# teamtomo/torch-motion-correction

Hardware: NVIDIA B200
Metric: movies_per_second_estimate_plus_correct (higher is better)
Workload: dtype f32

## Files before the change

torch_motion_correction_b200/csrc/fourier.cu:

```cuda
#include "common.cuh"
#include <stdlib.h>
#include "fft_core.cuh"
#include "fft_core2.cuh"

namespace {

using tmcfft::pad_idx;
using tmcfft::padded_len;

constexpr int kThreads = 256;

__host__ __device__ constexpr int batch_for(int n) { return n >= 4096 ? 1 : (4096 / n > 16 ? 16 : 4096 / n); }

template <int N>
constexpr size_t fft_smem_bytes() {
  return 2ull * batch_for(N) * padded_len(N) * sizeof(float2);
}


inline bool pow2_n(int n) { return n >= 16 && n <= 8192 && (n & (n - 1)) == 0; }
inline int fft_size_for(int n) {
  if (pow2_n(n)) return n;
  if (n < 2) return 0;
  int m = 16;
// ... 716 lines not shown
                        rows_per_cta));
        } else {
          if (int e = enable_smem(poly::rows_forward_poly<2>, poly::smem_bytes)) return e;
          TMC_TIMED("rows_forward_poly<2>", stream,
                    poly::rows_forward_poly<2><<<grid, poly::kThreads, poly::smem_bytes, stream>>>(
                        image, h, w, mean_std, mask, jobs, frame_shifts, x_margin, ylo, yhi, ny, kx_count, px.tw, (float2*)tmp,
                        rows_per_cta));
        }
        return TMC_OK;
      }
    }
    if constexpr ((MM == 8192 || MM == 4096) && !BB) {
      if (yhi > ylo && job_mode == 2 && px.R == 1 && kx_count <= MM / 2 && use_real2n(MM)) {
        constexpr int NH = MM / 2;
        constexpr int B = fft2::Cfg<NH>::B;
        int rows_per_cta = B * 4;
        while (rows_per_cta > B && (long)tmc_div_up(yhi - ylo, rows_per_cta) * njobs < 148 * 8) rows_per_cta -= B;
        dim3 grid(tmc_div_up(yhi - ylo, rows_per_cta), njobs);
        constexpr size_t smem = rows_forward_real2n_smem_bytes<NH>();
        if (int e = enable_smem(rows_forward_real2n<NH>, smem)) return e;
        TMC_TIMED(MM == 8192 ? "rows_forward_real2n<4096>" : "rows_forward_real2n<2048>", stream,
                  rows_forward_real2n<NH><<<grid, fft2::kThreads, smem, stream>>>(image, h, w, mean_std, mask, jobs, frame_shifts, x_margin,
                                                                                   ylo, yhi, ny, kx_count, px.tw, (float2*)tmp,
                                                                                   rows_per_cta));
        return TMC_OK;
      }
    }
    if constexpr (use_fast_path<MM, BB>()) if (px.R == 1) {
      if (yhi > ylo) {
        constexpr int B = fft2::Cfg<MM>::B;
        int rows_per_cta = B * 4;
        while (rows_per_cta > B && (long)tmc_div_up(yhi - ylo, rows_per_cta) * njobs < 148 * 8) rows_per_cta -= B;
        dim3 grid(tmc_div_up(yhi - ylo, rows_per_cta), njobs);
        constexpr size_t smem = rows_forward_smem_bytes<MM>();
#define TMC_ROWS_FWD(MODE)                                                                                      \
  {                                                                                                             \
    if (int e = enable_smem(rows_forward_p2<MM, MODE>, smem)) return e;                                         \
    tmc_timing_begin(stream);                                                                                   \
    rows_forward_p2<MM, MODE><<<grid, fft2::kThreads, smem, stream>>>(image, h, w, mean_std, mask, jobs, frame_shifts, \
                                                                     x_margin, ylo, yhi, ny, kx_count, px.tw,          \
                                                                     (float2*)tmp, rows_per_cta);                      \
    tmc_timing_end(MM == 4096 ? "rows_forward_p2<4096>" : "rows_forward_p2", stream);                            \
  }
        if (job_mode == 1) TMC_ROWS_FWD(1) else if (job_mode == 2) TMC_ROWS_FWD(2) else TMC_ROWS_FWD(0)
#undef TMC_ROWS_FWD
        tmc_count_launch();
      }
      return TMC_OK;
    }
    const size_t smem = fft_smem_bytes<MM>() + (px.R > 1 ? 2ull * batch_for(MM) * kx_count * sizeof(float2) : 0);
    if (smem > kMaxSmem) {
      tmc_set_error("rfft2_band: band of %d bins too wide for the decimated row transform of length %d", kx_count, nx);
      return TMC_ERR_UNSUPPORTED;
    }
    if (int e = enable_smem(rows_forward_kernel<MM, BB>, smem)) return e;
    dim3 grid(tmc_div_up(yhi - ylo, batch_for(MM)), njobs);
    if (yhi > ylo) {
      TMC_TIMED("rows_forward_kernel", stream, rows_forward_kernel<MM, BB><<<grid, kThreads, smem, stream>>>(
          image, h, w, mean_std, mask, jobs, frame_shifts, x_margin, ylo, yhi, ny, kx_count, px, (float2*)tmp));
    }
    return TMC_OK;
  });
}

}


TMC_API int tmc_fft_supported_length(int n) {
  if (fft_size_for(n) > 0) return 1;
  const int R = decimation_for(n);
  if (R == 0) return 0;
  return decimated_full_fits(n) ? 1 : 2;
}

TMC_API long tmc_fft_plan_elems(int n_total) {
  const int R = decimation_for(n_total);
  if (R == 0) return 0;
  const int n = n_total / R;
  const int m = fft_size_for(n);
  return m == n ? (long)m : 2l * m + n;
}

TMC_API int tmc_fft_plan_init(int n_total, void* plan, cudaStream_t stream) {
  TMC_CHECK_ARG(plan, "fft_plan_init: null pointer");
  const int R = decimation_for(n_total);
  if (R == 0) {
    tmc_set_error("fft_plan_init: transform length %d is not supported", n_total);
    return TMC_ERR_UNSUPPORTED;
  }
  const int n = n_total / R;
  const int m = fft_size_for(n);
  float2* tw = (float2*)plan;
  TMC_TIMED("twiddle_kernel", stream, twiddle_kernel<<<tmc_div_up(m, 128), 128, 0, stream>>>(m, tw));
  if (m != n) {
    float2* chirp = tw + m;
    float2* bhat = chirp + n;
    TMC_TIMED("chirp_kernel", stream, chirp_kernel<<<tmc_div_up(m, 128), 128, 0, stream>>>(n, m, chirp, bhat));
    AxisPlan p;
    p.tw = tw;
    p.chirp = nullptr;
    p.bhat = nullptr;
    p.n = m;
    p.R = 1;
    p.n_total = m;
    int rc = dispatch_fft(m, "fft_plan_init", [&](auto M, auto) {
      constexpr int MM = decltype(M)::value;
      if (int e = enable_smem(c2c_rows_kernel<MM, false>, fft_smem_bytes<MM>())) return e;
      TMC_TIMED("c2c_rows_kernel", stream, c2c_rows_kernel<MM, false><<<1, kThreads, fft_smem_bytes<MM>(), stream>>>(bhat, 1, p, bhat));
      return TMC_OK;
    });
    if (rc) return rc;
  }
  TMC_CHECK_LAUNCH("tmc_fft_plan_init");
  return TMC_OK;
}

TMC_API int tmc_fft_c2c_rows(const void* in, int rows, int n, const void* plan, void* out, cudaStream_t stream) {
  TMC_CHECK_ARG(in && out && plan && rows >= 1, "fft_c2c_rows: bad arguments");
  TMC_CHECK_ARG(fft_size_for(n) > 0, "fft_c2c_rows: full transforms need lengths up to 4096 or powers of two up to 8192, got %d", n);
  AxisPlan p = make_axis_plan(plan, n);
  int rc = dispatch_fft(n, "fft_c2c_rows", [&](auto M, auto BLU) {
    constexpr int MM = decltype(M)::value;
    constexpr bool BB = decltype(BLU)::value;
    if (int e = enable_smem(c2c_rows_kernel<MM, BB>, fft_smem_bytes<MM>())) return e;
    TMC_TIMED("c2c_rows_kernel", stream, c2c_rows_kernel<MM, BB><<<tmc_div_up(rows, batch_for(MM)), kThreads, fft_smem_bytes<MM>(), stream>>>(
        (const float2*)in, rows, p, (float2*)out));
    return TMC_OK;
  });
  if (rc) return rc;
  TMC_CHECK_LAUNCH("tmc_fft_c2c_rows");
  return TMC_OK;
}

TMC_API int tmc_rfft2_band(const float* image, int t, int h, int w, const float* mean_std, const float* mask, int ny, int nx,
                           const int* jobs, int njobs, int job_mode, const int* frame_shifts, int x_margin, int ylo, int yhi,
                           int kx_count, int ky_count, int ky_start, const float* weight, const void* plan_x,
                           const void* plan_y, void* tmp, void* out, cudaStream_t stream) {
  TMC_CHECK_ARG(image && jobs && plan_x && plan_y && tmp && out, "rfft2_band: null pointer");
  TMC_CHECK_ARG(job_mode >= 0 && job_mode <= 2, "rfft2_band: job_mode must be 0 (generic), 1 (mask powers 1,2 of one frame) or 2 (two frames)");
  TMC_CHECK_ARG(njobs >= 0 && t >= 1 && h >= ny && w >= nx, "rfft2_band: window (%d,%d) larger than image (%d,%d)", ny, nx, h, w);
  TMC_CHECK_ARG(0 <= ylo && ylo <= yhi && yhi <= ny, "rfft2_band: bad row support [%d,%d)", ylo, yhi);
  TMC_CHECK_ARG(x_margin >= 0 && 2 * x_margin <= nx, "rfft2_band: bad x_margin %d", x_margin);
  TMC_CHECK_ARG(kx_count >= 1 && kx_count <= nx / 2 + 1 && ky_count >= 1 && ky_count <= ny, "rfft2_band: bad band box");
  if (njobs == 0) return TMC_OK;
  const AxisPlan px = make_axis_plan(plan_x, nx), py = make_axis_plan(plan_y, ny);
  int rc = rfft2_rows(image, h, w, mean_std, mask, ny, nx, jobs, njobs, job_mode, frame_shifts, x_margin, ylo, yhi, kx_count,
                      px, tmp, stream);
  if (rc) return rc;
  TMC_CHECK_LAUNCH("tmc_rfft2_band(rows)");
  rc = dispatch_fft(ny, "rfft2_band", [&](auto M, auto BLU) {
    constexpr int MM = decltype(M)::value;
    constexpr bool BB = decltype(BLU)::value;
    if constexpr (use_fast_path<MM, BB>()) if (py.R == 1) {
      if (int e = enable_smem(cols_forward_p2<MM>, fft2::Cfg<MM>::smem_bytes)) return e;
      dim3 grid(tmc_div_up(kx_count, fft2::Cfg<MM>::B), 2 * njobs);
      TMC_TIMED(sized_label<MM>("cols_forward_p2<4096>", "cols_forward_p2<1024>", "cols_forward_p2"), stream, cols_forward_p2<MM><<<grid, fft2::kThreads, fft2::Cfg<MM>::smem_bytes, stream>>>(
          (const float2*)tmp, ylo, yhi, kx_count, ky_count, ky_start, weight, py.tw, (float2*)out));
      return TMC_OK;
    }
    const size_t smem = fft_smem_bytes<MM>() + (py.R > 1 ? 1ull * batch_for(MM) * ky_count * sizeof(float2) : 0);
    if (smem > kMaxSmem) {
      tmc_set_error("rfft2_band: band of %d bins too wide for the decimated column transform of length %d", ky_count, ny);
      return TMC_ERR_UNSUPPORTED;
    }
    if (int e = enable_smem(cols_forward_kernel<MM, BB>, smem)) return e;
    dim3 grid(tmc_div_up(kx_count, batch_for(MM)), 2 * njobs);
    TMC_TIMED("cols_forward_kernel", stream, cols_forward_kernel<MM, BB><<<grid, kThreads, smem, stream>>>(
                  (const float2*)tmp, ylo, yhi, kx_count, ky_count, ky_start, weight, py, (float2*)out));
    return TMC_OK;
  });
  if (rc) return rc;
  TMC_CHECK_LAUNCH("tmc_rfft2_band(cols)");
  return TMC_OK;
}

__global__ void integer_shifts_kernel(const float* __restrict__ field, int t, float scale, int* __restrict__ shifts,
                                      int* __restrict__ not_integer) {
  const int f = blockIdx.x * blockDim.x + threadIdx.x;
  if (f >= t) return;
  const float sy = scale * field[f], sx = scale * field[t + f];
  const float ry = rintf(sy), rx = rintf(sx);
  shifts[2 * f] = (int)ry;
  shifts[2 * f + 1] = (int)rx;
  if (!(fabsf(sy - ry) <= 1e-4f && fabsf(sx - rx) <= 1e-4f && fabsf(ry) < 1e6f && fabsf(rx) < 1e6f)) *not_integer = 1;
}

TMC_API int tmc_integer_shifts(const float* field, int t, float scale, int* shifts, int* not_integer, cudaStream_t stream) {
  TMC_CHECK_ARG(field && shifts && not_integer && t >= 1, "integer_shifts: bad arguments");
  TMC_CUDA(cudaMemsetAsync(not_integer, 0, sizeof(int), stream));
  TMC_TIMED("integer_shifts_kernel", stream, integer_shifts_kernel<<<tmc_div_up(t, 128), 128, 0, stream>>>(field, t, scale, shifts, not_integer));
  TMC_CHECK_LAUNCH("tmc_integer_shifts");
  return TMC_OK;
}

TMC_API int tmc_xc_pair_products(const void* spec, const int* ref_plane, const int* cur_plane, int nitems, long plane_elems,
                                 void* out, cudaStream_t stream) {
  TMC_CHECK_ARG(spec && ref_plane && cur_plane && out && nitems >= 0 && plane_elems >= 1, "xc_pair_products: bad arguments");
  if (nitems == 0) return TMC_OK;
  dim3 grid((unsigned)(tmc_div_up(plane_elems, 256) < 64 ? tmc_div_up(plane_elems, 256) : 64), nitems);
  TMC_TIMED("xc_pair_product_kernel", stream, xc_pair_product_kernel<<<grid, 256, 0, stream>>>((const float2*)spec, ref_plane, cur_plane, plane_elems, (float2*)out));
  TMC_CHECK_LAUNCH("tmc_xc_pair_products");
  return TMC_OK;
}

TMC_API int tmc_xc_leave_one_out_products(const void* spec, int t, int g, long plane_elems, const int* delta_offsets,
                                          const int* deltas, int k_begin, int k_count, void* out, cudaStream_t stream) {
  TMC_CHECK_ARG(spec && delta_offsets && deltas && out && t >= 2 && g >= 1 && plane_elems >= 1,
                "xc_leave_one_out_products: bad arguments (need t >= 2)");
  TMC_CHECK_ARG(k_begin >= 0 && k_count >= 0 && k_begin + k_count <= t, "xc_leave_one_out_products: bad frame range");
  if (k_count == 0) return TMC_OK;
  dim3 grid(tmc_div_up(plane_elems, 128), g);
  TMC_TIMED("xc_leave_one_out_kernel", stream, xc_leave_one_out_kernel<<<grid, 128, 0, stream>>>((const float2*)spec, t, g, plane_elems, delta_offsets, deltas,
                                                    k_begin, k_count, (float2*)out));
  TMC_CHECK_LAUNCH("tmc_xc_leave_one_out_products");
  return TMC_OK;
}

TMC_API int tmc_xc_peak_partials(int ny, int nx) {
  const int R = decimation_for(nx);
  if (R == 0) return -1;
  const int m = fft_size_for(nx / R);
  if (R == 1 && m == nx && m >= 256) {
    const int b = 256 / (m / 16) > 0 ? 256 / (m / 16) : 1;
    if (m == 8192 || m == 4096) {
      const int bh = 256 / (m / 32) > 0 ? 256 / (m / 32) : 1;
      return tmc_div_up(ny, bh * kRowIters);
    }
    return tmc_div_up(ny, 2 * b * kRowIters);
  }
  return tmc_div_up(ny, 2 * batch_for(m));
}

TMC_API int tmc_xc_peaks(const void* prod, int nitems, int ny, int nx, int kx_count, int ky_count, int ky_start,
                         int sub_pixel, const void* plan_x, const void* plan_y, void* tmp, void* partial, float* shifts,
                         cudaStream_t stream) {
  TMC_CHECK_ARG(prod && plan_x && plan_y && tmp && partial && shifts, "xc_peaks: null pointer");
  TMC_CHECK_ARG(kx_count >= 1 && kx_count <= nx / 2 + 1 && ky_count >= 1 && ky_count <= ny, "xc_peaks: bad band box");
  if (nitems == 0) return TMC_OK;
  const AxisPlan px = make_axis_plan(plan_x, nx), py = make_axis_plan(plan_y, ny);
  int rc = dispatch_fft(ny, "xc_peaks", [&](auto M, auto BLU) {
    constexpr int MM = decltype(M)::value;
    constexpr bool BB = decltype(BLU)::value;
    if constexpr (use_fast_path<MM, BB>()) if (py.R == 1) {
      if (int e = enable_smem(cols_inverse_p2<MM>, fft2::Cfg<MM>::smem_bytes)) return e;
      dim3 grid(tmc_div_up(kx_count, fft2::Cfg<MM>::B), nitems);
      TMC_TIMED(sized_label<MM>("cols_inverse_p2<4096>", "cols_inverse_p2<1024>", "cols_inverse_p2"), stream, cols_inverse_p2<MM><<<grid, fft2::kThreads, fft2::Cfg<MM>::smem_bytes, stream>>>(
          (const float2*)prod, kx_count, ky_count, ky_start, py.tw, (float2*)tmp));
      return TMC_OK;
    }
    if (int e = enable_smem(cols_inverse_kernel<MM, BB>, fft_smem_bytes<MM>())) return e;
    dim3 grid(tmc_div_up(kx_count, batch_for(MM)), nitems);
    TMC_TIMED("cols_inverse_kernel", stream, cols_inverse_kernel<MM, BB><<<grid, kThreads, fft_smem_bytes<MM>(), stream>>>((const float2*)prod, kx_count, ky_count, ky_start,
                                                                                 py, (float2*)tmp));
    return TMC_OK;
  });
  if (rc) return rc;
  TMC_CHECK_LAUNCH("tmc_xc_peaks(cols)");
  int nparts = tmc_xc_peak_partials(ny, nx);
  rc = dispatch_fft(nx, "xc_peaks", [&](auto M, auto BLU) {
    constexpr int MM = decltype(M)::value;
    constexpr bool BB = decltype(BLU)::value;
    if constexpr ((MM == 8192 || MM == 4096) && !BB) {
      if (px.R == 1 && kx_count <= MM / 4 && use_real2n(MM)) {
        constexpr int NH = MM / 2;
        if (int e = enable_smem(rows_inverse_argmax_real2n<NH>, rows_inverse_real2n_smem_bytes<NH>())) return e;
        nparts = tmc_div_up(ny, rows_per_cta_inverse_real2n<NH>());
        dim3 grid(nparts, nitems);
        TMC_TIMED(MM == 8192 ? "rows_inverse_argmax_real2n<4096>" : "rows_inverse_argmax_real2n<2048>", stream,
                  rows_inverse_argmax_real2n<NH><<<grid, fft2::kThreads, rows_inverse_real2n_smem_bytes<NH>(), stream>>>(
                      (const float2*)tmp, ny, kx_count, px.tw, (PeakCandidate*)partial));
        return TMC_OK;
      }
      nparts = tmc_div_up(ny, rows_per_cta_inverse<MM>());
    }
    if constexpr (MM == 1024 && !BB) {
      if (kx_count <= 128 && use_poly() && px.R == 1) {
        if (int e = enable_smem(poly::rows_inverse_argmax_poly, poly::smem_bytes)) return e;
        dim3 grid(nparts, nitems);
        TMC_TIMED("rows_inverse_argmax_poly", stream, poly::rows_inverse_argmax_poly<<<grid, poly::kThreads, poly::smem_bytes, stream>>>((const float2*)tmp, ny, kx_count, px.tw,
                                                                                         (PeakCandidate*)partial));
        return TMC_OK;
      }
    }
    if constexpr (use_fast_path<MM, BB>()) if (px.R == 1) {
      if (int e = enable_smem(rows_inverse_argmax_p2<MM>, rows_inverse_smem_bytes<MM>())) return e;
      dim3 grid(nparts, nitems);
      TMC_TIMED(sized_label<MM>("rows_inverse_argmax_p2<4096>", "rows_inverse_argmax_p2<1024>", "rows_inverse_argmax_p2"), stream, rows_inverse_argmax_p2<MM><<<grid, fft2::kThreads, rows_inverse_smem_bytes<MM>(), stream>>>(
          (const float2*)tmp, ny, kx_count, px.tw, (PeakCandidate*)partial));
      return TMC_OK;
    }
    if (int e = enable_smem(rows_inverse_argmax_kernel<MM, BB>, fft_smem_bytes<MM>())) return e;
    dim3 grid(nparts, nitems);
    TMC_TIMED("rows_inverse_argmax_kernel", stream, rows_inverse_argmax_kernel<MM, BB><<<grid, kThreads, fft_smem_bytes<MM>(), stream>>>((const float2*)tmp, ny, kx_count, px,
                                                                                        (PeakCandidate*)partial));
    return TMC_OK;
  });
  if (rc) return rc;
  TMC_CHECK_LAUNCH("tmc_xc_peaks(rows)");
  TMC_TIMED("peak_finalize_kernel", stream, peak_finalize_kernel<<<nitems, 128, 0, stream>>>((const float2*)tmp, (const PeakCandidate*)partial, nparts, ny, nx,
                                                   kx_count, sub_pixel, shifts));
  TMC_CHECK_LAUNCH("tmc_xc_peaks(finalize)");
  return TMC_OK;
}

namespace {

int irfft2_cols(const void* spec, int nitems, int ny, int KX, int KY, int ky_start, const AxisPlan& py, void* tmp,
                cudaStream_t stream, const char* who) {
  return dispatch_fft(ny, who, [&](auto M, auto BLU) {
    constexpr int MM = decltype(M)::value;
// ... 202 lines not shown
```

torch_motion_correction_b200/csrc/fourier_p2.cuh:

```cuda
#pragma once


__device__ __forceinline__ void cp_async_f32(float* smem_dst, const float* gmem_src) {
  const unsigned dst = (unsigned)__cvta_generic_to_shared(smem_dst);
  asm volatile("cp.async.ca.shared.global [%0], [%1], 4;\n" ::"r"(dst), "l"(gmem_src));
}
__device__ __forceinline__ void cp_async_commit_and_wait() {
  asm volatile("cp.async.commit_group;\n" ::);
  asm volatile("cp.async.wait_group 0;\n" ::: "memory");
}

template <int N>
constexpr size_t rows_forward_smem_bytes() {
  return fft2::Cfg<N>::smem_bytes + 3ull * fft2::Cfg<N>::B * N * sizeof(float);
}

template <int N, int MODE>
__global__ void __launch_bounds__(fft2::kThreads, N == 4096 ? 2 : 1)
rows_forward_p2(const float* __restrict__ image, int H, int W, const float* __restrict__ mean_std,
                const float* __restrict__ mask, const int* __restrict__ jobs, const int* __restrict__ frame_shifts,
                int x_margin, int ylo, int yhi, int NY, int KX, const float2* __restrict__ tw, float2* __restrict__ tmp,
                int rows_per_cta) {
  using C = fft2::Cfg<N>;
  using P = fft2::Plan<N>;
  extern __shared__ float2 smem[];
  const fft2::Smem<N> sm(smem);
  fft2::load_twiddles<N>(sm, tw);
  const int seq = threadIdx.x / C::TPS, j = threadIdx.x % C::TPS;
  float2* myseq = sm.data + seq * C::STRIDE;
  float* stage_a = reinterpret_cast<float*>(smem + C::B * C::STRIDE + 64 + C::TW_HI);
  float* stage_b = stage_a + C::B * N;
  float* stage_m = stage_b + C::B * N;
  const int job = blockIdx.y;
  const int fa = jobs[job * 6 + 0], ea = jobs[job * 6 + 1], fb = jobs[job * 6 + 2], eb = jobs[job * 6 + 3];
  const int y0 = jobs[job * 6 + 4], x0 = jobs[job * 6 + 5];
  float mean = 0.f, inv_std = 1.f;
  if (mean_std != nullptr) {
    mean = __ldg(mean_std);
    inv_std = 1.0f / __ldg(mean_std + 1);
  }
  const Window wa = make_window(image, fa, y0, x0, frame_shifts, H, W, ylo, yhi, N, x_margin);
  const Window wb = make_window(image, fb >= 0 ? fb : fa, y0, x0, frame_shifts, H, W, ylo, yhi, N, x_margin);
  const float* img_a = wa.fast_base(W);
  const bool has_b = fb >= 0;
  const bool separate_b = has_b && (MODE == 2 || (MODE == 0 && fb != fa));
  const float* img_b = wb.fast_base(W);
  const int row_begin = ylo + blockIdx.x * rows_per_cta;
  const int row_end = min(yhi, row_begin + rows_per_cta);
  float2* plane_a = tmp + (long)(2 * job) * NY * KX;
  float2* plane_b = plane_a + (long)NY * KX;

  auto prefetch = [&](int row0) {
    const int y = row0 + seq;
    if (y < row_end) {
#pragma unroll
      for (int e = 0; e < C::VPT; ++e) {
        const int x = P::First::in_index(j, e / P::First::R, e % P::First::R);
        const int slot = e * fft2::kThreads + threadIdx.x;
        cp_async_f32(stage_a + slot, wa.wrap ? wa.wrapped(y, x, H, W) : img_a + (long)y * W + x);
        if (separate_b) cp_async_f32(stage_b + slot, wb.wrap ? wb.wrapped(y, x, H, W) : img_b + (long)y * W + x);
        if (mask) cp_async_f32(stage_m + slot, mask + (long)y * N + x);
      }
    }
  };
  prefetch(row_begin);
  __syncthreads();
  for (int row0 = row_begin; row0 < row_end; row0 += C::B) {
    const int y = row0 + seq;
    const bool active = y < row_end;
    cp_async_commit_and_wait();
    float2 v[C::VPT];
#pragma unroll
    for (int e = 0; e < C::VPT; ++e) {
      float2 z = make_float2(0.f, 0.f);
      if (active) {
        const int slot = e * fft2::kThreads + threadIdx.x;
        const float m = mask ? stage_m[slot] : 1.0f;
        const float pa = (stage_a[slot] - mean) * inv_std;
        if (MODE == 1) {
          z.x = pa * m;
          z.y = z.x * m;
        } else if (MODE == 2) {
          z.x = pa * m;
          if (has_b) z.y = (stage_b[slot] - mean) * inv_std * m;
        } else {
          float va = pa;
          for (int k = 0; k < ea; ++k) va *= m;
          z.x = va;
          if (has_b) {
            float vb = separate_b ? (stage_b[slot] - mean) * inv_std : pa;
            for (int k = 0; k < eb; ++k) vb *= m;
            z.y = vb;
          }
        }
      }
      v[e] = z;
    }
    if (row0 + C::B < row_end) prefetch(row0 + C::B);
    fft2::fft_regs_to_regs<N>(sm, myseq, j, v);
    __syncthreads();
    P::Last::store(myseq, j, v);
    __syncthreads();
    if (active) {
      for (int k = j; k < KX; k += C::TPS) {
        const float2 zk = myseq[fft2::pad_idx(k)];
        const float2 zn = myseq[fft2::pad_idx(k == 0 ? 0 : N - k)];
        plane_a[(long)y * KX + k] = make_float2(0.5f * (zk.x + zn.x), 0.5f * (zk.y - zn.y));
        if (has_b) plane_b[(long)y * KX + k] = make_float2(0.5f * (zk.y + zn.y), -0.5f * (zk.x - zn.x));
      }
    }
    __syncthreads();
  }
}

__device__ __forceinline__ void cp_async_f32x2_any(float2* smem_dst, const float2* gmem_src) {
  const unsigned dst = (unsigned)__cvta_generic_to_shared(smem_dst);
  asm volatile("cp.async.ca.shared.global [%0], [%1], 8;\n" ::"r"(dst), "l"(gmem_src));
}

template <int N>
constexpr size_t rows_forward_real2n_smem_bytes() {
  return fft2::Cfg<N>::smem_bytes + 2ull * fft2::Cfg<N>::B * N * sizeof(float2);
}

template <int N>
__global__ void __launch_bounds__(fft2::kThreads, N >= 2048 ? 2 : 1)
rows_forward_real2n(const float* __restrict__ image, int H, int W, const float* __restrict__ mean_std,
                    const float* __restrict__ mask, const int* __restrict__ jobs, const int* __restrict__ frame_shifts,
                    int x_margin, int ylo, int yhi, int NY, int KX, const float2* __restrict__ tw2n,
                    float2* __restrict__ tmp, int rows_per_cta) {
  using C = fft2::Cfg<N>;
  using P = fft2::Plan<N>;
  extern __shared__ float2 smem[];
  const fft2::Smem<N> sm(smem);
  for (int i = threadIdx.x; i < 64 + C::TW_HI; i += fft2::kThreads)
    sm.tw_lo[i] = i < 64 ? __ldg(tw2n + 2 * i) : __ldg(tw2n + 2 * (i - 64) * 64);
  const int seq = threadIdx.x / C::TPS, j = threadIdx.x % C::TPS;
  float2* myseq = sm.data + seq * C::STRIDE;
  float2* stage_p = smem + C::B * C::STRIDE + 64 + C::TW_HI;
  float2* stage_m = stage_p + C::B * N;
  const int job = blockIdx.y;
  const int fa = jobs[job * 6 + 0], fb = jobs[job * 6 + 2];
  const int y0 = jobs[job * 6 + 4], x0 = jobs[job * 6 + 5];
  float mean = 0.f, inv_std = 1.f;
  if (mean_std != nullptr) {
    mean = __ldg(mean_std);
    inv_std = 1.0f / __ldg(mean_std + 1);
  }
  const Window wa = make_window(image, fa, y0, x0, frame_shifts, H, W, ylo, yhi, 2 * N, x_margin);
  const Window wb = make_window(image, fb >= 0 ? fb : fa, y0, x0, frame_shifts, H, W, ylo, yhi, 2 * N, x_margin);
  const int halves = fb >= 0 ? 2 : 1;
  const int row_begin = ylo + blockIdx.x * rows_per_cta;
  const int row_end = min(yhi, row_begin + rows_per_cta);
  const int nunits = row_end > row_begin ? ((row_end - row_begin + C::B - 1) / C::B) * halves : 0;
  float2* plane_a = tmp + (long)(2 * job) * NY * KX;

  auto prefetch = [&](int u) {
    const int y = row_begin + (u / halves) * C::B + seq;
    if (y >= row_end) return;
    const bool second = (u % halves) == 1;
    const Window& wd = second ? wb : wa;
    const float* row = wd.fast_base(W) + (long)y * W;
    const bool pair_ok = !wd.wrap && (reinterpret_cast<uintptr_t>(row) & 7) == 0;
#pragma unroll
    for (int e = 0; e < C::VPT; ++e) {
      const int x = 2 * P::First::in_index(j, e / P::First::R, e % P::First::R);
      const int slot = e * fft2::kThreads + threadIdx.x;
      if (pair_ok) {
        cp_async_f32x2_any(stage_p + slot, reinterpret_cast<const float2*>(row + x));
      } else {
        float* dst = reinterpret_cast<float*>(stage_p + slot);
        cp_async_f32(dst, wd.wrap ? wd.wrapped(y, x, H, W) : row + x);
        cp_async_f32(dst + 1, wd.wrap ? wd.wrapped(y, x + 1, H, W) : row + x + 1);
      }
      if (mask && !second) cp_async_f32x2_any(stage_m + slot, reinterpret_cast<const float2*>(mask + (long)y * (2 * N) + x));
    }
  };
  if (nunits > 0) prefetch(0);
  __syncthreads();
  for (int u = 0; u < nunits; ++u) {
    const int y = row_begin + (u / halves) * C::B + seq;
    const bool active = y < row_end;
    const bool second = (u % halves) == 1;
    cp_async_commit_and_wait();
    float2 v[C::VPT];
#pragma unroll
    for (int e = 0; e < C::VPT; ++e) {
      float2 z = make_float2(0.f, 0.f);
      if (active) {
        const int slot = e * fft2::kThreads + threadIdx.x;
        const float2 px = stage_p[slot];
        const float2 m = mask ? stage_m[slot] : make_float2(1.f, 1.f);
        z.x = (px.x - mean) * inv_std * m.x;
        z.y = (px.y - mean) * inv_std * m.y;
      }
      v[e] = z;
    }
    if (u + 1 < nunits) prefetch(u + 1);
    fft2::fft_regs_to_regs<N>(sm, myseq, j, v);
    __syncthreads();
    P::Last::store(myseq, j, v);
    __syncthreads();
    if (active) {
      float2* plane = plane_a + (second ? (long)NY * KX : 0l);
      for (int k = j; k < KX; k += C::TPS) {
        const float2 zk = myseq[fft2::pad_idx(k)];
        const float2 zn = myseq[fft2::pad_idx(k == 0 ? 0 : N - k)];
        const float2 ev = make_float2(0.5f * (zk.x + zn.x), 0.5f * (zk.y - zn.y));
        const float2 od = make_float2(0.5f * (zk.y + zn.y), -0.5f * (zk.x - zn.x));
        plane[(long)y * KX + k] = cadd(ev, cmul(__ldg(tw2n + k), od));
      }
    }
    __syncthreads();
  }
}

template <int N>
__global__ void __launch_bounds__(fft2::kThreads)
cols_forward_p2(const float2* __restrict__ tmp, int ylo, int yhi, int KX, int KY, int ky_start,
                const float* __restrict__ weight, const float2* __restrict__ tw, float2* __restrict__ out) {
  using C = fft2::Cfg<N>;
  using P = fft2::Plan<N>;
  extern __shared__ float2 smem[];
  const fft2::Smem<N> sm(smem);
  fft2::load_twiddles<N>(sm, tw);
  const int seq = threadIdx.x % C::B, j = threadIdx.x / C::B;
  float2* myseq = sm.data + seq * C::STRIDE;
  const long plane = blockIdx.y;
  const int kx = blockIdx.x * C::B + seq;
  const bool active = kx < KX;
  const float2* src = tmp + plane * N * KX + kx;
  float2 v[C::VPT];
#pragma unroll
  for (int g = 0; g < P::First::G; ++g)
#pragma unroll
    for (int r = 0; r < P::First::R; ++r) {
      const int y = P::First::in_index(j, g, r);
      v[g * P::First::R + r] = (active && y >= ylo && y < yhi) ? src[(long)y * KX] : make_float2(0.f, 0.f);
    }
  __syncthreads();
  fft2::fft_regs_to_regs<N>(sm, myseq, j, v);
  if (!active) return;
  float2* dst = out + plane * KY * KX + kx;
#pragma unroll
  for (int g = 0; g < P::Last::G; ++g)
#pragma unroll
    for (int r = 0; r < P::Last::R; ++r) {
      const int ky = P::Last::out_index(j, g, r);
      const int kyb = (ky - ky_start) & (N - 1);
      if (kyb < KY) {
        float2 val = P::Last::result(v, g, r);
        if (weight) {
          const float wgt = __ldg(weight + (long)kyb * KX + kx);
          val.x *= wgt;
          val.y *= wgt;
        }
        dst[(long)kyb * KX] = val;
      }
    }
}

template <int N>
__global__ void __launch_bounds__(fft2::kThreads)
cols_inverse_p2(const float2* __restrict__ in, int KX, int KY, int ky_start, const float2* __restrict__ tw,
                float2* __restrict__ tmp) {
  using C = fft2::Cfg<N>;
  using P = fft2::Plan<N>;
  extern __shared__ float2 smem[];
  const fft2::Smem<N> sm(smem);
  fft2::load_twiddles<N>(sm, tw);
  const int seq = threadIdx.x % C::B, j = threadIdx.x / C::B;
  float2* myseq = sm.data + seq * C::STRIDE;
  const long item = blockIdx.y;
  const int kx = blockIdx.x * C::B + seq;
  const bool active = kx < KX;
  const float2* src = in + item * KY * KX + kx;
  float2 v[C::VPT];
#pragma unroll
  for (int g = 0; g < P::First::G; ++g)
#pragma unroll
    for (int r = 0; r < P::First::R; ++r) {
      const int y = P::First::in_index(j, g, r);
      const int kyb = (y - ky_start) & (N - 1);
      float2 z = make_float2(0.f, 0.f);
      if (active && kyb < KY) {
        const float2 c = src[(long)kyb * KX];
        z = make_float2(c.y, c.x);
      }
      v[g * P::First::R + r] = z;
    }
  __syncthreads();
  fft2::fft_regs_to_regs<N>(sm, myseq, j, v);
  if (!active) return;
  float2* dst = tmp + item * N * KX + kx;
#pragma unroll
  for (int g = 0; g < P::Last::G; ++g)
#pragma unroll
    for (int r = 0; r < P::Last::R; ++r) {
      const float2 val = P::Last::result(v, g, r);
      dst[(long)P::Last::out_index(j, g, r) * KX] = make_float2(val.y, val.x);
    }
}


__device__ __forceinline__ void cp_async_f32x2(float2* smem_dst, const float2* gmem_src) {
  const unsigned dst = (unsigned)__cvta_generic_to_shared(smem_dst);
  asm volatile("cp.async.ca.shared.global [%0], [%1], 8;\n" ::"r"(dst), "l"(gmem_src));
}

constexpr int kRowIters = 4;

template <int N>
__host__ __device__ constexpr int rows_per_cta_inverse() {
  return 2 * fft2::Cfg<N>::B * kRowIters;
}

template <int N>
constexpr size_t rows_inverse_smem_bytes() {
  return fft2::Cfg<N>::smem_bytes + 2ull * fft2::Cfg<N>::B * N * sizeof(float2);
}

template <int N>
__device__ __forceinline__ int c2r_source_index(int i, int KX) {
  if (i < KX) return i;
  const int k = N - i;
  return (k < KX && 2 * k != N) ? k : -1;
}

template <int N>
__device__ __forceinline__ float2 c2r_pack(float2 ca, float2 cb, int i, int KX) {
  if (i < KX) {
    if (i == 0 || 2 * i == N) return make_float2(cb.x, ca.x);
    return make_float2(ca.y + cb.x, ca.x - cb.y);
  }
  return make_float2(cb.x - ca.y, ca.x + cb.y);
}

template <int N, typename Consume>
__device__ __forceinline__ void rows_inverse_driver(const float2* __restrict__ src, int NY, int KX,
                                                    const float2* __restrict__ tw, float2* smem, Consume&& consume) {
  using C = fft2::Cfg<N>;
  using P = fft2::Plan<N>;
  const fft2::Smem<N> sm(smem);
  fft2::load_twiddles<N>(sm, tw);
  const int seq = threadIdx.x / C::TPS, j = threadIdx.x % C::TPS;
  float2* myseq = sm.data + seq * C::STRIDE;
  float2* stage_a = smem + C::B * C::STRIDE + 64 + C::TW_HI;
  float2* stage_b = stage_a + C::B * N;
  auto row_of = [&](int it) { return (int)blockIdx.x * rows_per_cta_inverse<N>() + (it * C::B + seq) * 2; };
  auto prefetch = [&](int it) {
    const int ya = row_of(it);
    if (ya >= NY) return;
    const float2* rowa = src + (long)ya * KX;
    const bool has_b = ya + 1 < NY;
#pragma unroll
    for (int e = 0; e < C::VPT; ++e) {
      constexpr int R = P::First::R;
      const int lo = (e / R) * C::TPS + (e % R) * P::First::NBR;
      if (lo >= KX && lo + C::TPS <= N - KX + 1) continue;
      const int k = c2r_source_index<N>(P::First::in_index(j, e / R, e % R), KX);
      if (k >= 0) {
        const int slot = e * fft2::kThreads + threadIdx.x;
        cp_async_f32x2(stage_a + slot, rowa + k);
        if (has_b) cp_async_f32x2(stage_b + slot, rowa + KX + k);
      }
    }
  };
  prefetch(0);
  __syncthreads();
  for (int it = 0; it < kRowIters; ++it) {
    const int ya = row_of(it);
    const bool active = ya < NY;
    const bool has_b = ya + 1 < NY;
    cp_async_commit_and_wait();
    float2 v[C::VPT];
#pragma unroll
    for (int e = 0; e < C::VPT; ++e) {
      constexpr int R = P::First::R;
      float2 z = make_float2(0.f, 0.f);
      const int lo = (e / R) * C::TPS + (e % R) * P::First::NBR;
      if (active && !(lo >= KX && lo + C::TPS <= N - KX + 1)) {
        const int i = P::First::in_index(j, e / R, e % R);
        if (c2r_source_index<N>(i, KX) >= 0) {
          const int slot = e * fft2::kThreads + threadIdx.x;
          z = c2r_pack<N>(stage_a[slot], has_b ? stage_b[slot] : make_float2(0.f, 0.f), i, KX);
        }
      }
      v[e] = z;
    }
    if (it + 1 < kRowIters) prefetch(it + 1);
    fft2::fft_regs_to_regs<N>(sm, myseq, j, v);
    if (active) consume(ya, has_b, j, v);
    __syncthreads();
  }
}

template <int N>
__global__ void __launch_bounds__(fft2::kThreads, N == 4096 ? 3 : 1)
rows_inverse_argmax_p2(const float2* __restrict__ tmp, int NY, int KX, const float2* __restrict__ tw,
                       PeakCandidate* __restrict__ partial) {
  using P = fft2::Plan<N>;
  extern __shared__ float2 smem[];
  const long item = blockIdx.y;
  float best = -INFINITY;
  int best_idx = 0x7fffffff;
  rows_inverse_driver<N>(tmp + item * NY * KX, NY, KX, tw, smem, [&](int ya, bool has_b, int j, const float2* v) {
#pragma unroll
    for (int r = 0; r < P::Last::R; ++r)
#pragma unroll
      for (int g = 0; g < P::Last::G; ++g) {
        const float val = P::Last::result(v, g, r).y;
        if (val > best) {
          best = val;
          best_idx = ya * N + P::Last::out_index(j, g, r);
        }
      }
    if (has_b) {
#pragma unroll
      for (int r = 0; r < P::Last::R; ++r)
#pragma unroll
        for (int g = 0; g < P::Last::G; ++g) {
          const float val = P::Last::result(v, g, r).x;
          if (val > best) {
            best = val;
            best_idx = (ya + 1) * N + P::Last::out_index(j, g, r);
          }
        }
    }
  });
#pragma unroll
  for (int o = 16; o > 0; o >>= 1) {
    const float ov = __shfl_xor_sync(0xffffffffu, best, o);
    const int oi = __shfl_xor_sync(0xffffffffu, best_idx, o);
    if (better(ov, oi, best, best_idx)) {
      best = ov;
      best_idx = oi;
    }
  }
  __shared__ float sval[fft2::kThreads / 32];
  __shared__ int sidx[fft2::kThreads / 32];
  if ((threadIdx.x & 31) == 0) {
    sval[threadIdx.x >> 5] = best;
    sidx[threadIdx.x >> 5] = best_idx;
  }
  __syncthreads();
  if (threadIdx.x == 0) {
    for (int i = 1; i < fft2::kThreads / 32; ++i)
      if (better(sval[i], sidx[i], best, best_idx)) {
        best = sval[i];
        best_idx = sidx[i];
      }
    PeakCandidate c;
    c.val = best;
    c.idx = best_idx;
    partial[item * gridDim.x + blockIdx.x] = c;
  }
}

template <int N>
__host__ __device__ constexpr int rows_per_cta_inverse_real2n() {
  return fft2::Cfg<N>::B * kRowIters;
// ... 351 lines not shown
```

Baseline: 51.65.

## Make forward column FFT persistent over groups with cp.async prefetch staging

The forward column FFT kernel now handles several column groups per CTA, up to four when N<=4096. While it transforms the current group, it prefetches the next group's column data into a shared-memory staging buffer with cp.async. The goal is to hide global-load latency behind FFT compute and to reuse the twiddle load across groups. In exchange it uses more shared memory, raises the minimum blocks per SM in launch bounds, and launches fewer CTAs, which could reduce parallelism on small problems.

```diff
diff --git a/torch_motion_correction_b200/csrc/fourier.cu b/torch_motion_correction_b200/csrc/fourier.cu
--- a/torch_motion_correction_b200/csrc/fourier.cu
+++ b/torch_motion_correction_b200/csrc/fourier.cu
@@ -892,10 +892,11 @@
     constexpr int MM = decltype(M)::value;
     constexpr bool BB = decltype(BLU)::value;
     if constexpr (use_fast_path<MM, BB>()) if (py.R == 1) {
-      if (int e = enable_smem(cols_forward_p2<MM>, fft2::Cfg<MM>::smem_bytes)) return e;
-      dim3 grid(tmc_div_up(kx_count, fft2::Cfg<MM>::B), 2 * njobs);
-      TMC_TIMED(sized_label<MM>("cols_forward_p2<4096>", "cols_forward_p2<1024>", "cols_forward_p2"), stream, cols_forward_p2<MM><<<grid, fft2::kThreads, fft2::Cfg<MM>::smem_bytes, stream>>>(
-          (const float2*)tmp, ylo, yhi, kx_count, ky_count, ky_start, weight, py.tw, (float2*)out));
+      constexpr size_t smem = cols_forward_smem_bytes<MM>();
+      if (int e = enable_smem(cols_forward_p2<MM>, smem)) return e;
+      const long ngroups = (long)tmc_div_up(kx_count, fft2::Cfg<MM>::B) * 2 * njobs;
+      TMC_TIMED(sized_label<MM>("cols_forward_p2<4096>", "cols_forward_p2<1024>", "cols_forward_p2"), stream, cols_forward_p2<MM><<<tmc_div_up(ngroups, cols_forward_groups<MM>()), fft2::kThreads, smem, stream>>>(
+          (const float2*)tmp, ylo, yhi, kx_count, ky_count, ky_start, ngroups, weight, py.tw, (float2*)out));
       return TMC_OK;
     }
     const size_t smem = fft_smem_bytes<MM>() + (py.R > 1 ? 1ull * batch_for(MM) * ky_count * sizeof(float2) : 0);
diff --git a/torch_motion_correction_b200/csrc/fourier_p2.cuh b/torch_motion_correction_b200/csrc/fourier_p2.cuh
--- a/torch_motion_correction_b200/csrc/fourier_p2.cuh
+++ b/torch_motion_correction_b200/csrc/fourier_p2.cuh
@@ -8,6 +8,11 @@
 __device__ __forceinline__ void cp_async_commit_and_wait() {
   asm volatile("cp.async.commit_group;\n" ::);
   asm volatile("cp.async.wait_group 0;\n" ::: "memory");
+}
+
+__device__ __forceinline__ void cp_async_f32x2(float2* smem_dst, const float2* gmem_src) {
+  const unsigned dst = (unsigned)__cvta_generic_to_shared(smem_dst);
+  asm volatile("cp.async.ca.shared.global [%0], [%1], 8;\n" ::"r"(dst), "l"(gmem_src));
 }
 
 template <int N>
@@ -216,48 +221,90 @@
 }
 
 template <int N>
-__global__ void __launch_bounds__(fft2::kThreads)
-cols_forward_p2(const float2* __restrict__ tmp, int ylo, int yhi, int KX, int KY, int ky_start,
+__host__ __device__ constexpr bool cols_forward_staged() {
+  return N <= 4096;
+}
+
+template <int N>
+__host__ __device__ constexpr int cols_forward_groups() {
+  return cols_forward_staged<N>() ? 4 : 1;
+}
+
+template <int N>
+constexpr size_t cols_forward_smem_bytes() {
+  return fft2::Cfg<N>::smem_bytes + (cols_forward_staged<N>() ? (size_t)fft2::Cfg<N>::VPT * fft2::kThreads * sizeof(float2) : 0);
+}
+
+template <int N>
+__global__ void __launch_bounds__(fft2::kThreads, cols_forward_staged<N>() ? 3 : 2)
+cols_forward_p2(const float2* __restrict__ tmp, int ylo, int yhi, int KX, int KY, int ky_start, long ngroups,
                 const float* __restrict__ weight, const float2* __restrict__ tw, float2* __restrict__ out) {
+  constexpr bool STAGED = cols_forward_staged<N>();
   using C = fft2::Cfg<N>;
   using P = fft2::Plan<N>;
   extern __shared__ float2 smem[];
   const fft2::Smem<N> sm(smem);
   fft2::load_twiddles<N>(sm, tw);
+  float2* stage = smem + C::B * C::STRIDE + 64 + C::TW_HI;
   const int seq = threadIdx.x % C::B, j = threadIdx.x / C::B;
   float2* myseq = sm.data + seq * C::STRIDE;
-  const long plane = blockIdx.y;
-  const int kx = blockIdx.x * C::B + seq;
-  const bool active = kx < KX;
-  const float2* src = tmp + plane * N * KX + kx;
-  float2 v[C::VPT];
-#pragma unroll
-  for (int g = 0; g < P::First::G; ++g)
-#pragma unroll
-    for (int r = 0; r < P::First::R; ++r) {
-      const int y = P::First::in_index(j, g, r);
-      v[g * P::First::R + r] = (active && y >= ylo && y < yhi) ? src[(long)y * KX] : make_float2(0.f, 0.f);
-    }
-  __syncthreads();
-  fft2::fft_regs_to_regs<N>(sm, myseq, j, v);
-  if (!active) return;
-  float2* dst = out + plane * KY * KX + kx;
-#pragma unroll
-  for (int g = 0; g < P::Last::G; ++g)
-#pragma unroll
-    for (int r = 0; r < P::Last::R; ++r) {
-      const int ky = P::Last::out_index(j, g, r);
-      const int kyb = (ky - ky_start) & (N - 1);
-      if (kyb < KY) {
-        float2 val = P::Last::result(v, g, r);
-        if (weight) {
-          const float wgt = __ldg(weight + (long)kyb * KX + kx);
-          val.x *= wgt;
-          val.y *= wgt;
+  const int gx = (KX + C::B - 1) / C::B;
+  const long u0 = (long)blockIdx.x * cols_forward_groups<N>();
+  const int nu = (int)min((long)cols_forward_groups<N>(), ngroups - u0);
+  auto prefetch = [&](long u) {
+    if constexpr (!STAGED) return;
+    const long plane = u / gx;
+    const int kx = (int)(u - plane * gx) * C::B + seq;
+    if (kx >= KX) return;
+    const float2* src = tmp + plane * N * KX + kx;
+#pragma unroll
+    for (int g = 0; g < P::First::G; ++g)
+#pragma unroll
+      for (int r = 0; r < P::First::R; ++r) {
+        const int y = P::First::in_index(j, g, r);
+        if (y >= ylo && y < yhi) cp_async_f32x2(stage + (g * P::First::R + r) * fft2::kThreads + threadIdx.x, src + (long)y * KX);
+      }
+  };
+  prefetch(u0);
+  for (int i = 0; i < nu; ++i) {
+    const long u = u0 + i;
+    const long plane = u / gx;
+    const int kx = (int)(u - plane * gx) * C::B + seq;
+    const bool active = kx < KX;
+    if (STAGED) cp_async_commit_and_wait();
+    const float2* src = tmp + plane * N * KX + kx;
+    float2 v[C::VPT];
+#pragma unroll
+    for (int g = 0; g < P::First::G; ++g)
+#pragma unroll
+      for (int r = 0; r < P::First::R; ++r) {
+        const int y = P::First::in_index(j, g, r);
+        v[g * P::First::R + r] = !(active && y >= ylo && y < yhi) ? make_float2(0.f, 0.f)
+                                 : STAGED ? stage[(g * P::First::R + r) * fft2::kThreads + threadIdx.x]
+                                          : src[(long)y * KX];
+      }
+    if (i + 1 < nu) prefetch(u + 1);
+    __syncthreads();
+    fft2::fft_regs_to_regs<N>(sm, myseq, j, v);
+    if (!active) continue;
+    float2* dst = out + plane * KY * KX + kx;
+#pragma unroll
+    for (int g = 0; g < P::Last::G; ++g)
+#pragma unroll
+      for (int r = 0; r < P::Last::R; ++r) {
+        const int ky = P::Last::out_index(j, g, r);
+        const int kyb = (ky - ky_start) & (N - 1);
+        if (kyb < KY) {
+          float2 val = P::Last::result(v, g, r);
+          if (weight) {
+            const float wgt = __ldg(weight + (long)kyb * KX + kx);
+            val.x *= wgt;
+            val.y *= wgt;
+          }
+          dst[(long)kyb * KX] = val;
         }
-        dst[(long)kyb * KX] = val;
-      }
-    }
+      }
+  }
 }
 
 template <int N>
@@ -302,11 +349,6 @@
     }
 }
 
-
-__device__ __forceinline__ void cp_async_f32x2(float2* smem_dst, const float2* gmem_src) {
-  const unsigned dst = (unsigned)__cvta_generic_to_shared(smem_dst);
-  asm volatile("cp.async.ca.shared.global [%0], [%1], 8;\n" ::"r"(dst), "l"(gmem_src));
-}
 
 constexpr int kRowIters = 4;
 
```

After: 49.13 (median of 6 runs). 4.9% lower.
